# CovertLab/Lens

Measured on AMD Instinct MI355X. Metric: agent-steps/sec (whole node) at 1M agents; FP64 % peak; stencil HBM GB/s, higher is better.
Workload: dtype f64; 1 GPU; BASELINE config 4: 1M agents + 4096x4096 diffusion_field lattice; agents=1000000, agents_end=1000000, agents_start=1000000, integrator=dopri5, exchange=sorted, parallelism=row-bands x1, agents_in_bin_order=True, coupled_passes=False, stencil_mode=fma, halo=0

## Files before the change

include/vk_kinetics.h:

```cpp
#ifndef VK_KINETICS_H
#define VK_KINETICS_H

#include <stdint.h>

#ifdef __cplusplus
extern "C" {
#endif

#define VK_ABI_VERSION 1

typedef void *vk_stream_t;
typedef struct vk_table vk_table;

enum vk_status {
    VK_OK = 0,
    VK_ERR_ARG = 1,
    VK_ERR_HIP = 2,
    VK_ERR_LIMIT = 3,
    VK_ERR_NOMEM = 4
};

enum vk_agent_status {
    VK_AGENT_OK = 0,
    VK_AGENT_MAX_STEPS = 1,
// ... 69 lines not shown
int vk_step_dopri5_multi(const vk_table *t, int64_t n_agents, int64_t ld, double dt, int32_t n_steps,
                         const vk_ode_opts *opts, const double *params, double *conc, const double *m2c,
                         double *h_state, double *flux, int64_t step_flux, int64_t *counts,
                         int64_t step_counts, int32_t *status, int32_t *nsteps, int64_t step_nsteps,
                         vk_stream_t stream);


#define VK_UNIFORM_BLOCKS 512
int vk_field_uniform(const double *fields, int32_t n_fields, int64_t field_stride,
                     int32_t ny, int32_t row_lo, int32_t row_hi, double *summary,
                     int32_t *scratch, vk_stream_t stream);

int vk_diffuse(double *field, double *work0, double *work1, int32_t n_fields,
               int64_t field_stride, int32_t ny, int32_t row_lo, int32_t row_hi,
               int32_t lo_min, int32_t hi_max, int32_t edge_top, int32_t edge_bot,
               int32_t sub_begin, int32_t sub_count, int32_t n_sub, double coeff_dt,
               const double *uniform, vk_stream_t stream);

enum { VK_PART_ALL = 0, VK_PART_INTERIOR = 1, VK_PART_EDGES = 2 };
int vk_diffuse_part(double *field, double *work0, double *work1, int32_t n_fields,
                    int64_t field_stride, int32_t ny, int32_t row_lo, int32_t row_hi,
                    int32_t lo_min, int32_t hi_max, int32_t edge_top, int32_t edge_bot,
                    int32_t sub_begin, int32_t sub_count, int32_t n_sub, double coeff_dt,
                    const double *uniform, int32_t part, int32_t interior_passes,
                    vk_stream_t stream);

int vk_diffuse_delta(double *field, double *work0, double *work1, double *delta, int32_t n_fields,
                     int64_t field_stride, int32_t ny, int32_t row_lo, int32_t row_hi, int32_t lo_min,
                     int32_t hi_max, int32_t edge_top, int32_t edge_bot, int32_t sub_begin,
                     int32_t sub_count, int32_t n_sub, double coeff_dt, const double *uniform,
                     vk_stream_t stream);

int vk_diffuse_coupled(double *field, double *work0, double *work1, int32_t n_fields,
                       int64_t field_stride, int32_t ny, int32_t rows, int32_t n_sub, double coeff_dt,
                       const double *uniform, const int32_t *bin_lin, const int32_t *seg, int32_t nseg,
                       int64_t n_agents, const int32_t *gather_row, double *conc, int64_t conc_ld,
                       const int32_t *count_row, const int64_t *counts, int64_t counts_ld,
                       double binvol_avogadro, vk_stream_t stream);

enum { VK_BUF_FIELD = 0, VK_BUF_WORK0 = 1, VK_BUF_WORK1 = 2 };
enum { VK_PASS_SINGLE = 0, VK_PASS_WL3, VK_PASS_WL6, VK_PASS_WL6NT, VK_PASS_PS, VK_PASS_PS10,
       VK_PASS_PS10_ALIGNED, VK_PASS_PS10_STRIPS, VK_PASS_SP };
enum { VK_PLAN_COUPLED = 1, VK_PLAN_COUPLED_AGENTS = 2 };
typedef struct vk_pass {
    int32_t k, src, dst, f0;
    int32_t lo, hi, in_lo, in_hi, gap_lo, gap_hi;
    int32_t kernel, couple, copy_back;
} vk_pass;
int vk_diffuse_plan(int32_t row_lo, int32_t row_hi, int32_t lo_min, int32_t hi_max, int32_t edge_top,
                    int32_t edge_bot, int32_t sub_begin, int32_t sub_count, int32_t n_sub, int32_t part,
                    int32_t interior_passes, int32_t coupled, vk_pass *out, int32_t capacity,
                    int32_t *n_passes);

int vk_set_stencil_depth(int32_t k);

int vk_set_stencil_kernel(int32_t variant, int32_t rows);

int vk_set_stencil_mode(int32_t mode);

int vk_timestamp(uint64_t *out, int32_t idx, vk_stream_t stream);

int vk_copy_stream(const double *src, double *dst, int64_t n, vk_stream_t stream);

int64_t vk_wall_clock_khz(void);

int vk_gather(const double *fields, int64_t field_stride, const int32_t *bin_lin,
              int64_t n_agents, const int32_t *map_field, const int32_t *map_row,
              int32_t n_map, double *dst, int64_t ld, vk_stream_t stream);

int vk_exchange_sorted(double *fields, int64_t field_stride, const int32_t *occ_bin,
                       const int32_t *occ_ptr, const int32_t *occ_agent, int32_t n_occ,
                       const int64_t *counts, int64_t ld, const int32_t *map_count,
                       const int32_t *map_field, int32_t n_map, double binvol_avogadro,
                       vk_stream_t stream);

int vk_exchange_atomic(double *fields, int64_t field_stride, const int32_t *bin_lin,
                       int64_t n_agents, const int64_t *counts, int64_t ld,
                       const int32_t *map_count, const int32_t *map_field, int32_t n_map,
                       double binvol_avogadro, vk_stream_t stream);

int vk_bin_sites(const double *loc, int64_t n_agents, int64_t ld, int32_t nx, int32_t ny,
                 double bound_x, double bound_y, int32_t row_offset, int32_t *bin_lin,
                 int32_t *ix_out, vk_stream_t stream);


enum vk_cell_row {
    VK_CELL_MASS = 0,
    VK_CELL_VOLUME = 1,
    VK_CELL_LENGTH = 2,
    VK_CELL_SURFACE_AREA = 3,
    VK_CELL_PROTEIN = 4,
    VK_CELL_ANGLE = 5,
    VK_CELL_ROWS = 6
};

enum vk_growth_model {
    VK_GROWTH_PROTEIN = 0,
    VK_GROWTH_MASS = 1
};

enum vk_rng {
    VK_RNG_STREAM = 0,
    VK_RNG_PHILOX = 1
};

typedef struct vk_cell_params {
// ... 312 lines not shown
```

lens_amd/csrc/vk_lattice.hip:

```cpp

#include <math.h>
#include <stdint.h>

#include <algorithm>
#include <utility>
#include <vector>


#include "vk_bin.h"
#include "vk_internal.h"
#include "vk_pass_plan.h"
#include "vk_stencil_launch.h"

constexpr int ST_BX = 256;
constexpr int ST_RB = 16;

__global__ __launch_bounds__(ST_BX) void k_diffuse_substep(const double *__restrict__ src,
                                                           double *dst,
                                                           const double *f0,
                                                           int64_t field_stride, int ny, int lo, int hi,
                                                           int top_reflect, int bot_reflect, double coef,
                                                           const double *__restrict__ uniform, int delta_mode) {
    const int f = blockIdx.z;
    const int j = blockIdx.x * ST_BX + threadIdx.x;
    const int r0 = lo + blockIdx.y * ST_RB;
    if (j >= ny || r0 >= hi) return;
    const int r1 = min(r0 + ST_RB, hi);
    const double *s = src + (int64_t)f * field_stride;
    double *d = dst + (int64_t)f * field_stride;
    const double *g = f0 ? f0 + (int64_t)f * field_stride : nullptr;
    if (uniform && uniform[2 * f] == uniform[2 * f + 1]) {
        if (delta_mode)
            for (int r = r0; r < r1; ++r) d[(int64_t)r * ny + j] = 0.0;
        return;
    }
    const int jl = j > 0 ? j - 1 : 0;
    const int jr = j < ny - 1 ? j + 1 : ny - 1;
    const int ru = (r0 == top_reflect) ? r0 : r0 - 1;
    double up = s[(int64_t)ru * ny + j];
    double c = s[(int64_t)r0 * ny + j];
    for (int r = r0; r < r1; ++r) {
        const int rd = (r == bot_reflect) ? r : r + 1;
        const double down = s[(int64_t)rd * ny + j];
        const double left = s[(int64_t)r * ny + jl];
        const double right = s[(int64_t)r * ny + jr];
        const double lap = (((up + left) + (-4.0 * c)) + right) + down;
        double v = c + coef * lap;
        if (g) {
            const double base = g[(int64_t)r * ny + j];
            v = delta_mode ? v - base : base + (v - base);
        }
        d[(int64_t)r * ny + j] = v;
        up = c;
        c = down;
    }
}

// ... 25 lines not shown
    return prev;
}


__global__ void k_timestamp(uint64_t *out, int idx) {
    if (threadIdx.x == 0) out[idx] = wall_clock64();
}

extern "C" int vk_timestamp(uint64_t *out, int32_t idx, vk_stream_t stream) {
    if (!out || idx < 0) {
        vk::set_error("vk_timestamp: bad arguments");
        return VK_ERR_ARG;
    }
    hipLaunchKernelGGL(k_timestamp, dim3(1), dim3(64), 0, (hipStream_t)stream, out, idx);
    return vk::launch_check("k_timestamp");
}

typedef double vk_d2v __attribute__((ext_vector_type(2)));
__global__ __launch_bounds__(256) void k_copy_stream(const vk_d2v *__restrict__ s, vk_d2v *__restrict__ d, int64_t n) {
    const int64_t i = (int64_t)blockIdx.x * 256 + threadIdx.x;
    if (i < n) __builtin_nontemporal_store(s[i], d + i);
}

extern "C" int vk_copy_stream(const double *src, double *dst, int64_t n_doubles, vk_stream_t stream) {
    if (!src || !dst || n_doubles < 0 || (n_doubles & 1) || (((uintptr_t)src | (uintptr_t)dst) & 15)) {
        vk::set_error("vk_copy_stream: bad arguments (16-B aligned buffers of an even number of doubles)");
        return VK_ERR_ARG;
    }
    const int64_t n = n_doubles / 2;
    if (n == 0) return VK_OK;
    hipLaunchKernelGGL(k_copy_stream, dim3((unsigned)((n + 255) / 256)), dim3(256), 0, (hipStream_t)stream,
                       (const vk_d2v *)src, (vk_d2v *)dst, n);
    return vk::launch_check("k_copy_stream");
}

extern "C" int64_t vk_wall_clock_khz(void) {
    int dev = 0, khz = 0;
    if (hipGetDevice(&dev) != hipSuccess) return 0;
    if (hipDeviceGetAttribute(&khz, hipDeviceAttributeWallClockRate, dev) != hipSuccess) return 0;
    return khz;
}

__global__ __launch_bounds__(256) void k_copy_rows(const double *__restrict__ src, double *dst,
                                                   int64_t field_stride, int64_t off, int64_t count,
                                                   const double *__restrict__ uniform) {
    const int f = blockIdx.y;
    if (uniform && uniform[2 * f] == uniform[2 * f + 1]) return;
    const int64_t base = (int64_t)f * field_stride + off;
    for (int64_t i = (int64_t)blockIdx.x * blockDim.x + threadIdx.x; i < count; i += (int64_t)gridDim.x * blockDim.x)
        dst[base + i] = src[base + i];
}


static vk_plan::Settings stencil_settings() {
    return {g_stencil_mode, g_stencil_depth, g_stencil_kernel, g_stencil_rows};
}

struct PassArgs {
    double *buf[3];
    int nf;
    int64_t fs;
    int ny, top, bot, tile_rows;
    double coef;
    const double *uniform;
    const VkPsCouple *cp;
    hipStream_t stream;
};

static void launch_pass(const vk_pass &p, const PassArgs &a) {
    typedef void (*launcher)(VK_STENCIL_LAUNCH_ARGS);
    static const launcher launchers[] = {nullptr,        vk_launch_wl3,  vk_launch_wl6,          vk_launch_wl6nt,
                                         vk_launch_ps,   vk_launch_ps10, vk_launch_ps10_aligned, nullptr,
                                         vk_launch_sp};
    const double *src = a.buf[p.src], *f0 = p.f0 ? a.buf[VK_BUF_FIELD] : nullptr;
    double *dst = a.buf[p.dst];
    VkPsCouple c = {};
    if (a.cp) c = *a.cp, c.mode = p.couple;
    const VkPsCouple *cp = a.cp ? &c : nullptr;
    if (p.kernel == VK_PASS_SINGLE) {
        dim3 grid((a.ny + ST_BX - 1) / ST_BX, (p.hi - p.lo + ST_RB - 1) / ST_RB, a.nf);
        hipLaunchKernelGGL(k_diffuse_substep, grid, dim3(ST_BX), 0, a.stream, src, dst, f0, a.fs, a.ny, p.lo, p.hi, a.top,
                           a.bot, a.coef, a.uniform, 0);
    } else if (p.kernel == VK_PASS_PS10_STRIPS) {
        vk_launch_ps10_strips(p.k, a.stream, src, dst, f0, a.nf, a.fs, a.ny, p.lo, p.hi, p.in_lo, p.in_hi, a.top, a.bot,
                              a.coef, a.uniform, cp, a.tile_rows, p.gap_lo, p.gap_hi);
    } else {
        launchers[p.kernel](p.k, a.stream, src, dst, f0, a.nf, a.fs, a.ny, p.lo, p.hi, p.in_lo, p.in_hi, a.top, a.bot,
                            a.coef, a.uniform, cp, a.tile_rows);
    }
}

static int run_plan(const char *what, const vk_plan::Call &c, double *field, double *work0, double *work1, int32_t n_fields,
                    int64_t field_stride, int32_t ny, double coeff_dt, const double *uniform, const VkPsCouple *cp,
                    vk_stream_t stream) {
    const vk_plan::Settings st = stencil_settings();
    std::vector<vk_pass> passes;
    const char *why = "";
    int rc = vk_plan::plan(st, c, passes, &why);
    if (rc) {
        vk::set_error("%s: %s", what, why);
        return rc;
    }
    if (n_fields == 0) return VK_OK;
    const PassArgs a = {{field, work0, work1}, n_fields, field_stride, ny, c.edge_top ? c.lo_min : -1,
                        c.edge_bot ? c.hi_max - 1 : 0x7fffffff, st.rows, coeff_dt, uniform, cp, (hipStream_t)stream};
    for (const vk_pass &p : passes) {
        launch_pass(p, a);
        if ((rc = vk::launch_check(what))) return rc;
        if (p.copy_back) {
            const int64_t count = (int64_t)(c.row_hi - c.row_lo) * ny;
            const unsigned blocks = (unsigned)std::min<int64_t>(2048, (count + 255) / 256);
            hipLaunchKernelGGL(k_copy_rows, dim3(blocks, n_fields), dim3(256), 0, a.stream, work0, field, field_stride,
                               (int64_t)c.row_lo * ny, count, uniform);
            if ((rc = vk::launch_check("k_copy_rows"))) return rc;
        }
    }
    return VK_OK;
}

extern "C" int vk_diffuse_part(double *field, double *work0, double *work1, int32_t n_fields, int64_t field_stride,
                               int32_t ny, int32_t row_lo, int32_t row_hi, int32_t lo_min, int32_t hi_max,
                               int32_t edge_top, int32_t edge_bot, int32_t sub_begin, int32_t sub_count,
                               int32_t n_sub, double coeff_dt, const double *uniform, int32_t part,
                               int32_t interior_passes, vk_stream_t stream) {
    const vk_plan::Call c = {row_lo,    row_hi,    lo_min, hi_max, edge_top,        edge_bot,
                             sub_begin, sub_count, n_sub,  part,   interior_passes, 0};
    if (part != VK_PART_ALL && part != VK_PART_INTERIOR && part != VK_PART_EDGES) {
        vk::set_error("vk_diffuse_part: part must be VK_PART_ALL / _INTERIOR / _EDGES");
        return VK_ERR_ARG;
    }
    if (!field || n_fields < 0 || ny <= 0 || !vk_plan::geometry_ok(c) || (int64_t)hi_max * ny > field_stride) {
        vk::set_error("vk_diffuse: bad geometry");
        return VK_ERR_ARG;
    }
    if (!work0 || (n_sub > 2 && !work1)) {
        vk::set_error("vk_diffuse: work buffers required");
        return VK_ERR_ARG;
    }
    return run_plan("vk_diffuse", c, field, work0, work1, n_fields, field_stride, ny, coeff_dt, uniform, nullptr, stream);
}

extern "C" int vk_diffuse(double *field, double *work0, double *work1, int32_t n_fields,
                          int64_t field_stride, int32_t ny, int32_t row_lo, int32_t row_hi, int32_t lo_min,
                          int32_t hi_max, int32_t edge_top, int32_t edge_bot, int32_t sub_begin,
                          int32_t sub_count, int32_t n_sub, double coeff_dt, const double *uniform,
                          vk_stream_t stream) {
    return vk_diffuse_part(field, work0, work1, n_fields, field_stride, ny, row_lo, row_hi, lo_min, hi_max, edge_top,
                           edge_bot, sub_begin, sub_count, n_sub, coeff_dt, uniform, VK_PART_ALL, 0, stream);
}

extern "C" int vk_diffuse_plan(int32_t row_lo, int32_t row_hi, int32_t lo_min, int32_t hi_max, int32_t edge_top,
                               int32_t edge_bot, int32_t sub_begin, int32_t sub_count, int32_t n_sub, int32_t part,
                               int32_t interior_passes, int32_t coupled, vk_pass *out, int32_t capacity,
                               int32_t *n_passes) {
    const vk_plan::Call c = {row_lo,    row_hi,    lo_min, hi_max, edge_top,        edge_bot,
                             sub_begin, sub_count, n_sub,  part,   interior_passes, coupled};
    const bool whole_step = row_lo == 0 && lo_min == 0 && row_hi == hi_max && sub_begin == 0 && sub_count == n_sub &&
                            part == VK_PART_ALL;
    if (!n_passes || capacity < 0 || (capacity > 0 && !out) || part < VK_PART_ALL || part > VK_PART_EDGES ||
        coupled < 0 || coupled > VK_PLAN_COUPLED_AGENTS || (coupled && !whole_step) || !vk_plan::geometry_ok(c)) {
        vk::set_error("vk_diffuse_plan: bad arguments");
        return VK_ERR_ARG;
    }
    std::vector<vk_pass> passes;
    const char *why = "";
    const int rc = vk_plan::plan(stencil_settings(), c, passes, &why);
    if (rc) vk::set_error("vk_diffuse_plan: %s", why);
    *n_passes = (int32_t)passes.size();
    std::copy_n(passes.begin(), std::min<size_t>(passes.size(), (size_t)capacity), out);
    return rc;
}

extern "C" int vk_diffuse_coupled(double *field, double *work0, double *work1, int32_t n_fields,
                                  int64_t field_stride, int32_t ny, int32_t rows, int32_t n_sub, double coeff_dt,
                                  const double *uniform, const int32_t *bin_lin, const int32_t *seg, int32_t nseg,
                                  int64_t n_agents, const int32_t *gather_row, double *conc, int64_t conc_ld,
                                  const int32_t *count_row, const int64_t *counts, int64_t counts_ld,
                                  double binvol_avogadro, vk_stream_t stream) {
    if (!field || !work0 || !work1 || n_fields < 1 || ny <= 0 || rows <= 0 || n_sub < 0 ||
        (int64_t)rows * ny > field_stride || (int64_t)rows * ny >= INT32_MAX || n_agents < 0 ||
        n_agents >= INT32_MAX || nseg != (ny + 15) / 16 || (n_agents > 0 && (!bin_lin || !seg)) || !gather_row ||
        !count_row) {
        vk::set_error("vk_diffuse_coupled: bad arguments");
        return VK_ERR_ARG;
    }
    VkPsCouple cp = {};
    cp.bins = bin_lin;
    cp.seg = seg;
    cp.nseg = nseg;
    cp.n = (int32_t)n_agents;
    cp.gdst = conc;
    cp.gld = conc_ld;
    cp.counts = counts;
    cp.cld = counts_ld;
    cp.bva = binvol_avogadro;
    if (n_fields > VK_COUPLE_MAX_FIELDS) {
        vk::set_error("vk_diffuse_coupled: at most 8 planes");
        return VK_ERR_LIMIT;
    }
    for (int f = 0; f < n_fields; ++f) {
        if (gather_row[f] >= 127 || count_row[f] >= 127 || (gather_row[f] >= 0 && (!conc || conc_ld < n_agents)) ||
            (count_row[f] >= 0 && (!counts || counts_ld < n_agents))) {
            vk::set_error("vk_diffuse_coupled: bad gather / count rows");
            return VK_ERR_ARG;
        }
        cp.grow[f] = (int8_t)(gather_row[f] < 0 ? -1 : gather_row[f]);
        cp.crow[f] = (int8_t)(count_row[f] < 0 ? -1 : count_row[f]);
    }
    const vk_plan::Call c = {0, rows, 0, rows, 1, 1, 0, n_sub, n_sub, VK_PART_ALL, 0,
                             n_agents > 0 ? VK_PLAN_COUPLED_AGENTS : VK_PLAN_COUPLED};
    return run_plan("vk_diffuse_coupled", c, field, work0, work1, n_fields, field_stride, ny, coeff_dt, uniform, &cp, stream);
}

extern "C" int vk_diffuse_delta(double *field, double *work0, double *work1, double *delta, int32_t n_fields,
                                int64_t field_stride, int32_t ny, int32_t row_lo, int32_t row_hi, int32_t lo_min,
                                int32_t hi_max, int32_t edge_top, int32_t edge_bot, int32_t sub_begin,
                                int32_t sub_count, int32_t n_sub, double coeff_dt, const double *uniform,
                                vk_stream_t stream) {
    if (!delta || sub_count < 1 || sub_begin + sub_count != n_sub) {
        vk::set_error("vk_diffuse_delta: needs a delta buffer and the call must end at the last substep");
        return VK_ERR_ARG;
    }
    if (sub_count > 1) {
// ... 234 lines not shown
```

lens_amd/csrc/vk_pass_plan.h:

```cpp
#pragma once

#include <stdint.h>

#include <algorithm>
#include <vector>

#include "vk_kinetics.h"

namespace vk_plan {

struct Settings {
    int mode;
    int depth;
    int kernel;
    int rows;
};

struct Call {
    int row_lo, row_hi, lo_min, hi_max, edge_top, edge_bot, sub_begin, sub_count, n_sub, part, interior_passes, coupled;
};

inline bool geometry_ok(const Call &c) {
    return c.row_lo >= c.lo_min && c.row_hi <= c.hi_max && c.row_lo < c.row_hi && c.sub_begin >= 0 && c.sub_count >= 0 &&
           c.sub_begin + c.sub_count <= c.n_sub;
}

inline std::vector<int> odd_depths(int set_depth, int sub_count) {
    const int depth = set_depth == 10 ? 9 : std::min(set_depth | 1, 15);
    int passes = (sub_count + depth - 1) / depth;
    if ((passes & 1) != (sub_count & 1)) ++passes;
    std::vector<int> ks;
    for (int j = 0, left = passes; j < sub_count; --left) {
        const int rem = sub_count - j;
        int k = (rem + left - 1) / left;
        if ((k & 1) == 0) ++k;
        if (k > depth) k = depth;
        while (k > 1 && rem - k < left - 1) k -= 2;
        ks.push_back(k);
        j += k;
    }
    return ks;
}

inline int kernel_of(const Settings &s, int k, bool base, int couple, bool strip) {
    if (k == 1) return VK_PASS_SINGLE;
    if (s.mode == 1 && k <= 11 && ((k & 1) || k == 10)) {
        if (k != 10) return VK_PASS_PS;
        if (s.kernel == 40 && !strip && !couple) return VK_PASS_SP;
        return s.kernel == 70 && !strip ? VK_PASS_PS10_ALIGNED : VK_PASS_PS10;
    }
    if (k == 10 || ((s.kernel == 6 || s.kernel >= 20) && (k == 7 || k == 9 || k == 11))) return VK_PASS_WL6NT;
    return (s.kernel == 2 || base) ? VK_PASS_WL3 : VK_PASS_WL6;
}

inline int state_buffer(int j) { return j == 0 ? VK_BUF_FIELD : VK_BUF_WORK0 + ((j - 1) & 1); }

inline std::vector<int> ten_deep_buffers(const Settings &s, const Call &c, int P) {
    const bool ends_step = c.sub_begin + c.sub_count == c.n_sub;
    const int S = state_buffer(c.sub_begin);
    const int T = ends_step ? VK_BUF_FIELD : state_buffer(c.sub_begin + c.sub_count);
    const int cand[3] = {VK_BUF_WORK0, VK_BUF_WORK1, VK_BUF_FIELD};
    const int nc = (ends_step && s.mode == 1) ? 3 : 2;
    std::vector<int> dsts(P, -1);
    dsts[P - 1] = T;
    for (int p = P - 2; p >= 0; --p) {
        for (int i = 0; i < nc && dsts[p] < 0; ++i)
            if (cand[i] != dsts[p + 1] && (p > 0 || cand[i] != S)) dsts[p] = cand[i];
        if (dsts[p] < 0) return {};
// ... 21 lines not shown
        p.gap_lo = gap_lo, p.gap_hi = gap_hi;
        if (c.coupled == VK_PLAN_COUPLED_AGENTS)
            p.couple = (e - k + 1 == 0 ? 1 : 0) | (e == c.n_sub - 1 ? 2 : 0);
        p.kernel = gap_lo >= 0 ? VK_PASS_PS10_STRIPS : kernel_of(s, k, base, p.couple, strip);
        out.push_back(p);
    };
    const int P = c.sub_count / 10;
    std::vector<int> dsts;
    if (ten_block && P <= 64 && (!c.coupled || (s.mode == 1 && P >= 2))) dsts = ten_deep_buffers(s, c, P);
    if (!dsts.empty()) {
        const int m = (c.interior_passes <= 0 || c.interior_passes > P) ? P : c.interior_passes;
        for (int p = 0; p < P; ++p) {
            if (c.part == VK_PART_INTERIOR && p >= m) break;
            const int e = c.sub_begin + 10 * p + 9, grow = last - e;
            const int lo = std::max(c.lo_min, c.row_lo - grow), hi = std::min(c.hi_max, c.row_hi + grow);
            const int src = p ? dsts[p - 1] : state_buffer(c.sub_begin);
            const bool base = (s.mode != 1 || c.coupled) && ends_step && p == P - 1;
            const int ilo = halo_top ? c.row_lo + 10 * (p + 1) : lo, ihi = halo_bot ? c.row_hi - 10 * (p + 1) : hi;
            if (c.part == VK_PART_ALL || (c.part == VK_PART_EDGES && p >= m)) {
                add(10, e, src, dsts[p], base, lo, hi, false, -1, -1);
            } else if (c.part == VK_PART_INTERIOR) {
                if (ilo < ihi) add(10, e, src, dsts[p], base, ilo, ihi, false, -1, -1);
            } else if (halo_top && halo_bot && ilo < ihi && s.mode == 1) {
                add(10, e, src, dsts[p], base, lo, hi, true, ilo, ihi);
            } else {
                if (halo_top && lo < ilo) add(10, e, src, dsts[p], base, lo, ilo, true, -1, -1);
                if (halo_bot && ihi < hi) add(10, e, src, dsts[p], base, ihi, hi, true, -1, -1);
            }
        }
        return VK_OK;
    }
    if (c.part != VK_PART_ALL) {
        *why = "no 10-deep buffer plan for this block";
        return VK_ERR_LIMIT;
    }
    const std::vector<int> ks = odd_depths(s.depth, c.sub_count);
    if (c.coupled && (ks.size() < 2 || *std::min_element(ks.begin(), ks.end()) < 2)) {
        *why = "the step is not planned as two or more fused passes";
        return VK_ERR_LIMIT;
    }
    int j = c.sub_begin;
    for (int k : ks) {
        const int e = j + k - 1, grow = last - e;
        const bool final_pass = e == c.n_sub - 1, in_place = final_pass && j == 0;
        const int dst = in_place ? VK_BUF_WORK0 : (final_pass ? VK_BUF_FIELD : state_buffer(e + 1));
        add(k, e, state_buffer(j), dst, final_pass, std::max(c.lo_min, c.row_lo - grow),
            std::min(c.hi_max, c.row_hi + grow), false, -1, -1);
        out.back().copy_back = in_place;
        j += k;
    }
    return VK_OK;
}

}
```

lens_amd/lattice.py:

```python

from __future__ import annotations

import ctypes
from typing import Callable, Optional, Sequence

import torch

from lens_amd import native

N_A_LEGACY = 6.022140857e23


def n_substeps(timestep: float, dt_max: float = 0.01) -> int:
    t, dt, n = 0.0, min(timestep, dt_max), 0
    while t < timestep:
        t += dt
        n += 1
    return n


def whole_plane(lat) -> bool:
    return not (lat.pad_top or lat.pad_bot or not (lat.edge_top and lat.edge_bot))


def stencil_depth(k: int = 0) -> int:
    native.load()
    return native._lib.vk_set_stencil_depth(int(k))


def stencil_kernel(variant: int = -1, rows: int = -1) -> int:
    native.load()
    if int(variant) != -1 and int(variant) not in STENCIL_VARIANTS:
        raise ValueError('stencil kernel %d is not built (variants: %s)' % (variant, sorted(STENCIL_VARIANTS)))
    if int(rows) != -1 and not (int(rows) == 0 or 8 <= int(rows) <= 4096):
        raise ValueError('stencil tile rows must be 0 (auto) or 8..4096, got %d' % rows)
    return native._lib.vk_set_stencil_kernel(int(variant), int(rows))


STENCIL_VARIANTS = frozenset((2, 3, 6, 20, 40, 70))


def stencil_mode(mode=None) -> str:
    native.load()
    names = ('exact', 'fma')
    code = -1 if mode is None else names.index(mode)
    return names[native._lib.vk_set_stencil_mode(code)]


class Lattice:
    def __init__(self, molecules: Sequence[str], n_bins, bounds, depth: float, diffusion: float,
                 device=None, row_band=None, halo: int = 0, avogadro: float = N_A_LEGACY,
                 initial=None):
        native.load()
        self.molecules = list(molecules)
        self.n_bins = [int(n_bins[0]), int(n_bins[1])]
        self.bounds = [float(bounds[0]), float(bounds[1])]
        self.depth = float(depth)
        self.avogadro = float(avogadro)
        nx, ny = self.n_bins
        self.device = native.resolve_device(device)
        dx = self.bounds[0] / nx
        dy = self.bounds[1] / ny
        self.diffusion = diffusion / (dx * dy)
        self.diffusion_dt = 0.01
        self.bin_volume = (self.depth * self.bounds[0] * self.bounds[1]) * 1e-15 / (nx * ny)
        self.binvol_avogadro = self.bin_volume * self.avogadro
        lo, hi = (0, nx) if row_band is None else (int(row_band[0]), int(row_band[1]))
        if not (0 <= lo < hi <= nx):
            raise ValueError('bad row band %r' % (row_band,))
        self.row_lo_global, self.row_hi_global = lo, hi
        self.halo = int(halo)
        self.edge_top = lo == 0
        self.edge_bot = hi == nx
        if not (self.edge_top and self.edge_bot) and self.halo < 1:
            raise ValueError('a row band %r of %d rows needs halo >= 1 (got %d)' % ((lo, hi), nx, self.halo))
        if self.halo > hi - lo and not (self.edge_top and self.edge_bot):
            raise ValueError('halo (%d) deeper than the band (%d rows)' % (self.halo, hi - lo))
        h = self.halo
        self.pad_top = 0 if self.edge_top else h
        self.pad_bot = 0 if self.edge_bot else h
        self.rows_local = self.pad_top + (hi - lo) + self.pad_bot
        self.ny = ny
        nf = len(self.molecules)
        shape = (nf, self.rows_local, ny)
        self.fields = torch.zeros(shape, dtype=torch.float64, device=self.device)
        self.work0 = torch.empty(shape, dtype=torch.float64, device=self.device)
        self.work1 = torch.empty(shape, dtype=torch.float64, device=self.device)
        self.uniform = torch.empty(2 * max(nf, 1), dtype=torch.float64, device=self.device)
        self._uniform_scratch = torch.empty(max(nf, 1) * native.VK_UNIFORM_BLOCKS, dtype=torch.int32,
                                            device=self.device)
        if initial is not None:
            for f, m in enumerate(self.molecules):
                if m in initial:
                    self.set_field(m, initial[m])
        else:
            self.fields.fill_(1.0)

    @property
    def row_lo(self) -> int:
# ... 256 lines not shown
```

lens_amd/native.py:

```python

from __future__ import annotations

import ctypes
import os

import numpy as np

LIB_DIR = os.path.join(os.path.dirname(os.path.abspath(__file__)), 'lib')
LIB_PATH = os.environ.get('VK_KINETICS_LIB') or os.path.join(LIB_DIR, 'libvk_kinetics.so')

VK_OK, VK_ERR_ARG, VK_ERR_HIP, VK_ERR_LIMIT, VK_ERR_NOMEM = 0, 1, 2, 3, 4
VK_AGENT_MAX_STEPS, VK_AGENT_H_UNDERFLOW, VK_AGENT_NONFINITE = 1, 2, 4

EXPORTS = (
    'vk_abi_version', 'vk_last_error', 'vk_table_create', 'vk_table_destroy', 'vk_table_specialize',
    'vk_rate_fluxes', 'vk_step_euler', 'vk_step_dopri5', 'vk_step_dopri5_multi', 'vk_step_dopri5_gather', 'vk_field_uniform',
    'vk_diffuse', 'vk_diffuse_part', 'vk_diffuse_delta', 'vk_diffuse_coupled', 'vk_diffuse_plan', 'vk_set_stencil_depth', 'vk_set_stencil_kernel', 'vk_set_stencil_mode',
    'vk_timestamp', 'vk_wall_clock_khz', 'vk_copy_stream', 'vk_gather', 'vk_exchange_sorted',
    'vk_exchange_atomic', 'vk_bin_sites', 'vk_cell_step', 'vk_divide_scratch_bytes', 'vk_divide_plan',
    'vk_divide_gather', 'vk_divide_lineage', 'vk_divide_locations', 'vk_kremling_step',
    'vk_expression_step', 'vk_motility_step', 'vk_occupancy_scratch_bytes', 'vk_occupancy_sort',
    'vk_exchange_ordered', 'vk_contact_scratch_bytes', 'vk_contact_step',
    'vk_response_begin', 'vk_response_end', 'vk_response_cells', 'vk_exchange_ordered_mixed',
    'vk_exchange_atomic_f64', 'vk_population_scratch_bytes', 'vk_population_plan', 'vk_contact_step_channels',
    'vk_flagella_step', 'vk_flagella_counts', 'vk_divide_flagella',
    'vk_ssa_step', 'vk_ssa_propensities', 'vk_divide_counts', 'vk_ssa_flagella_target',
)

VK_CELL_MASS, VK_CELL_VOLUME, VK_CELL_LENGTH, VK_CELL_SURFACE_AREA, VK_CELL_PROTEIN, VK_CELL_ANGLE = range(6)
VK_CELL_ROWS = 6
(VK_MOTIL_N_METHYL, VK_MOTIL_ACTIVITY, VK_MOTIL_CHEY_P, VK_MOTIL_CCW_MOTOR_BIAS, VK_MOTIL_CCW_TO_CW,
 VK_MOTIL_MOTOR_STATE, VK_MOTIL_ANGLE, VK_MOTIL_THRUST, VK_MOTIL_TORQUE) = range(9)
VK_MOTIL_ROWS = 9
VK_FLAG_CHEY, VK_FLAG_CHEY_P, VK_FLAG_CW_BIAS, VK_FLAG_MOTILE_STATE, VK_FLAG_PMF = range(5)
VK_FLAG_ROWS = 5
VK_FLAGI_TARGET, VK_FLAGI_HAVE, VK_FLAGI_MASK = range(3)
VK_FLAGI_ROWS = 3
VK_FLAGELLA_MERGED, VK_FLAGELLA_SPLIT_DICT = 0, 1
VK_DIVIDE_FLAGELLA_DOMAIN = 0x666c6167656c6c61
VK_SSA_MAX_SPECIES, VK_SSA_MAX_REACTIONS, VK_SSA_MAX_ORDER = 64, 32, 255
VK_SSA_DOMAIN = 0x7373615f73746570
VK_SSA_DIVIDE_DOMAIN = 0x7373615f64697669
VK_SSA_MAX_EVENTS, VK_SSA_NONFINITE, VK_SSA_OVERFLOW, VK_SSA_BAD_KEY = 1, 2, 4, 8
VK_GROWTH_PROTEIN, VK_GROWTH_MASS = 0, 1
VK_RNG_STREAM, VK_RNG_PHILOX = 0, 1
VK_DIVIDE_SET, VK_DIVIDE_SPLIT, VK_DIVIDE_ZERO = 0, 1, 2
VK_UNIFORM_BLOCKS = 512
VK_PART_ALL, VK_PART_INTERIOR, VK_PART_EDGES = 0, 1, 2
VK_PLAN_COUPLED, VK_PLAN_COUPLED_AGENTS = 1, 2


class NativeError(RuntimeError):
    pass


_i32p = ctypes.POINTER(ctypes.c_int32)
_f64p = ctypes.POINTER(ctypes.c_double)
_vp = ctypes.c_void_p
_i32 = ctypes.c_int32
_i64 = ctypes.c_int64
_f64 = ctypes.c_double


class VkTableDesc(ctypes.Structure):
    _fields_ = [(n, ctypes.c_int32) for n in (
        'n_species', 'n_dyn', 'n_reactions', 'n_rate_laws', 'n_params', 'n_ext',
        'n_sets', 'n_members', 'n_upd', 'n_exch')] + [
        ('rl_reaction', _i32p), ('rl_enzyme', _i32p), ('rl_kcat', _i32p),
        ('rl_num_ptr', _i32p), ('rl_den_ptr', _i32p), ('set_ptr', _i32p),
        ('mem_species', _i32p), ('mem_param', _i32p), ('upd_ptr', _i32p),
# ... 37 lines not shown
class VkContactParams(ctypes.Structure):
    _fields_ = [(n, ctypes.c_int32) for n in ('iterations', 'gx', 'gy', 'reserved')] + [
        (n, ctypes.c_double) for n in ('stiffness', 'max_length', 'width', 'length', 'max_push', 'max_turn',
                                       'jitter', 'jitter_angle')] + [('seed', ctypes.c_uint64)]


class VkContactChannels(ctypes.Structure):
    _fields_ = [(n, ctypes.c_double) for n in ('height', 'space', 'spacer')] + [
        ('n_lines', ctypes.c_int32), ('reserved', ctypes.c_int32)]


class VkResponseTable(ctypes.Structure):
    _fields_ = [(n, ctypes.c_int32) for n in ('n_mol', 'n_porin', 'n_det', 'n_save', 'n_expr', 'n_flux', 'n_ext',
                                              'reserved')] + [
        (n, _vp) for n in ('mol_int_row', 'mol_ext_row', 'porin_row', 'porin_perm', 'det_row', 'det_thr',
                           'save_row', 'expr_row')] + [('avogadro', ctypes.c_double), ('volume_fl', ctypes.c_double)]


class VkSsaNet(ctypes.Structure):
    _fields_ = [(n, ctypes.c_int32) for n in ('n_species', 'n_reactions', 'max_order', 'n_inv')] + [
        (n, _vp) for n in ('react_ptr', 'react_species', 'react_order', 'stoich_ptr', 'stoich_species',
                           'stoich_delta', 'rates', 'inv')]


class VkPass(ctypes.Structure):
    _fields_ = [(n, ctypes.c_int32) for n in ('k', 'src', 'dst', 'f0', 'lo', 'hi', 'in_lo', 'in_hi', 'gap_lo',
                                              'gap_hi', 'kernel', 'couple', 'copy_back')]


_SIGS = {
    'vk_abi_version': ([], ctypes.c_int),
    'vk_last_error': ([], ctypes.c_char_p),
    'vk_table_create': ([ctypes.POINTER(VkTableDesc), ctypes.POINTER(_vp)], ctypes.c_int),
    'vk_table_destroy': ([_vp], ctypes.c_int),
    'vk_table_specialize': ([_vp, ctypes.c_char_p], ctypes.c_int),
    'vk_rate_fluxes': ([_vp, _i64, _i64, _vp, _vp, _vp, _vp], ctypes.c_int),
    'vk_step_euler': ([_vp, _i64, _i64, _f64, _vp, _vp, _vp, _vp, _vp, _vp, _vp, _vp], ctypes.c_int),
    'vk_step_dopri5': ([_vp, _i64, _i64, _f64, ctypes.POINTER(VkOdeOpts), _vp, _vp, _vp, _vp,
                        _vp, _vp, _vp, _vp, _vp, _vp], ctypes.c_int),
    'vk_step_dopri5_multi': ([_vp, _i64, _i64, _f64, _i32, ctypes.POINTER(VkOdeOpts), _vp, _vp, _vp, _vp, _vp,
                              _i64, _vp, _i64, _vp, _vp, _i64, _vp], ctypes.c_int),
    'vk_step_dopri5_gather': ([_vp, _i64, _i64, _f64, ctypes.POINTER(VkOdeOpts), _vp, _vp, _vp, _vp, _vp, _vp,
                               _vp, _vp, _vp, _i64, _vp, _vp, _vp, _i32, _vp], ctypes.c_int),
    'vk_field_uniform': ([_vp, _i32, _i64, _i32, _i32, _i32, _vp, _vp, _vp], ctypes.c_int),
    'vk_diffuse': ([_vp, _vp, _vp, _i32, _i64, _i32, _i32, _i32, _i32, _i32, _i32, _i32,
                    _i32, _i32, _i32, _f64, _vp, _vp], ctypes.c_int),
    'vk_diffuse_part': ([_vp, _vp, _vp, _i32, _i64, _i32, _i32, _i32, _i32, _i32, _i32, _i32,
                         _i32, _i32, _i32, _f64, _vp, _i32, _i32, _vp], ctypes.c_int),
    'vk_diffuse_delta': ([_vp, _vp, _vp, _vp, _i32, _i64, _i32, _i32, _i32, _i32, _i32, _i32, _i32,
                          _i32, _i32, _i32, _f64, _vp, _vp], ctypes.c_int),
    'vk_diffuse_coupled': ([_vp, _vp, _vp, _i32, _i64, _i32, _i32, _i32, _f64, _vp, _vp, _vp, _i32, _i64,
                            _i32p, _vp, _i64, _i32p, _vp, _i64, _f64, _vp], ctypes.c_int),
    'vk_diffuse_plan': ([_i32] * 12 + [ctypes.POINTER(VkPass), _i32, _i32p], ctypes.c_int),
    'vk_set_stencil_depth': ([_i32], ctypes.c_int),
    'vk_set_stencil_kernel': ([_i32, _i32], ctypes.c_int),
    'vk_set_stencil_mode': ([_i32], ctypes.c_int),
    'vk_timestamp': ([_vp, _i32, _vp], ctypes.c_int),
    'vk_wall_clock_khz': ([], ctypes.c_int64),
    'vk_copy_stream': ([_vp, _vp, _i64, _vp], ctypes.c_int),
    'vk_gather': ([_vp, _i64, _vp, _i64, _vp, _vp, _i32, _vp, _i64, _vp], ctypes.c_int),
    'vk_exchange_sorted': ([_vp, _i64, _vp, _vp, _vp, _i32, _vp, _i64, _vp, _vp, _i32, _f64, _vp],
                           ctypes.c_int),
    'vk_exchange_atomic': ([_vp, _i64, _vp, _i64, _vp, _i64, _vp, _vp, _i32, _f64, _vp], ctypes.c_int),
    'vk_bin_sites': ([_vp, _i64, _i64, _i32, _i32, _f64, _f64, _i32, _vp, _vp, _vp], ctypes.c_int),
    'vk_cell_step': ([ctypes.POINTER(VkCellParams), _i64, _i64, _vp, _vp, _vp, _vp, _vp, _vp, _vp, _vp],
                     ctypes.c_int),
    'vk_divide_scratch_bytes': ([_i64], ctypes.c_int64),
    'vk_divide_plan': ([_vp, _i64, _vp, _vp, _vp, _vp, _vp], ctypes.c_int),
    'vk_divide_gather': ([_i64, _vp, _vp, _vp, _i64, _vp, _i64, _i32, _i32, _i32, _vp], ctypes.c_int),
    'vk_divide_lineage': ([_i64, _vp, _vp, _vp, _vp, _vp, _vp, _vp, _vp, _vp, _vp], ctypes.c_int),
    'vk_divide_locations': ([_i64, _vp, _vp, _vp, _i64, _vp, _i64, _vp, _vp], ctypes.c_int),
    'vk_expression_step': ([_vp, _i64, _i64, _f64, _vp, _vp, _vp, _i32, _vp], ctypes.c_int),
    'vk_kremling_step': ([ctypes.POINTER(VkKremlingParams), _i64, _i64, _f64, _f64, _i32, _f64, _f64, _i32,
                          _vp, _vp, _f64, _vp, _vp, _vp, _vp, _vp, _vp], ctypes.c_int),
    'vk_motility_step': ([ctypes.POINTER(VkMotilityParams), _i64, _i64, _f64, _i32, _vp, _vp, _vp, _vp, _i32, _i32,
                          _f64, _f64, _vp, _vp, _vp, _vp], ctypes.c_int),
    'vk_flagella_step': ([ctypes.POINTER(VkMotilityParams), ctypes.POINTER(VkFlagellaParams), _i64, _i64, _f64, _i32,
                          _vp, _vp, _vp, _vp, _vp, _vp, _i32, _i32, _f64, _f64, _vp, _vp, _vp, _vp], ctypes.c_int),
    'vk_flagella_counts': ([_i64, _vp, _vp, _vp, _vp, _vp], ctypes.c_int),
    'vk_divide_flagella': ([_i64, _i64, _i64, _vp, _vp, _vp, _i64, _vp, _vp, _vp, _vp, _vp, _i64, _vp, _i32,
                            ctypes.c_uint64, ctypes.c_uint64, _i64, _vp], ctypes.c_int),
    'vk_ssa_step': ([ctypes.POINTER(VkSsaNet), _i64, _i64, _f64, _vp, _vp, ctypes.c_uint64, _vp, _i32, _vp, _vp, _vp],
                    ctypes.c_int),
    'vk_ssa_propensities': ([ctypes.POINTER(VkSsaNet), _i64, _i64, _vp, _vp, _vp], ctypes.c_int),
    'vk_divide_counts': ([_i64, _i64, _i64, _vp, _vp, _vp, _i64, _vp, _vp, _i64, _vp, _i32, ctypes.c_uint64,
                          ctypes.c_uint64, _i64, _vp], ctypes.c_int),
    'vk_ssa_flagella_target': ([_i64, _vp, _vp, _vp, _vp], ctypes.c_int),
    'vk_occupancy_scratch_bytes': ([_i64], ctypes.c_int64),
    'vk_occupancy_sort': ([_vp, _vp, _i64, _i64, _vp, _vp, _vp, _i64, _vp], ctypes.c_int),
    'vk_exchange_ordered': ([_vp, _i64, _vp, _vp, _i64, _vp, _i64, _vp, _vp, _i32, _f64, _vp], ctypes.c_int),
    'vk_contact_scratch_bytes': ([_i64, _i64], ctypes.c_int64),
    'vk_contact_step': ([ctypes.POINTER(VkContactParams), _i64, _i64, _vp, _vp, _vp, _vp, _vp, _vp, _i32, _i32,
                         _f64, _f64, _vp, _vp, _vp, _i64, _vp], ctypes.c_int),
    'vk_contact_step_channels': ([ctypes.POINTER(VkContactParams), _i64, _i64, _vp, _vp, _vp, _vp, _vp, _vp, _i32,
                                  _i32, _f64, _f64, _vp, _vp, _vp, _i64, ctypes.POINTER(VkContactChannels), _vp, _vp],
                                 ctypes.c_int),
    'vk_population_scratch_bytes': ([_i64], ctypes.c_int64),
    'vk_population_plan': ([_vp, _vp, _i64, _vp, _vp, _vp, _vp, _vp], ctypes.c_int),
    'vk_response_begin': ([ctypes.POINTER(VkResponseTable), _i64, _i64, _f64] + [_vp] * 14, ctypes.c_int),
    'vk_response_end': ([ctypes.POINTER(VkResponseTable), _i64, _i64] + [_vp] * 15, ctypes.c_int),
    'vk_response_cells': ([_i32, _i64, _i64, _vp, _vp, _vp, _vp, _vp, _vp, _vp, _vp, _vp], ctypes.c_int),
    'vk_exchange_ordered_mixed': ([_vp, _i64, _vp, _vp, _i64, _vp, _i64, _vp, _vp, _i32, _vp, _i64, _vp, _vp, _i32,
                                   _f64, _vp], ctypes.c_int),
    'vk_exchange_atomic_f64': ([_vp, _i64, _vp, _i64, _vp, _i64, _vp, _vp, _i32, _f64, _vp], ctypes.c_int),
}

# ... 94 lines not shown
```

Baseline: 793.7 million agent-steps/s.

## Split stencil passes into two row bands on a second stream with event dependencies

Adds a banded planning mode that splits each 10-step PS10 stencil pass into a top and a bottom row band. The bottom bands run on an extra non-blocking stream and wait on events from the previous top band, so the two bands' passes can overlap as a skewed wavefront. This targets the serialization and tail idle time between full-lattice passes on the whole-step 4096-row case. In exchange it adds event and stream overhead, extra halo-row reads at the band boundary, and a fallback path when graph capture or event limits prevent it.

```diff
diff --git a/include/vk_kinetics.h b/include/vk_kinetics.h
--- a/include/vk_kinetics.h
+++ b/include/vk_kinetics.h
@@ -145,6 +145,13 @@
                     int32_t interior_passes, int32_t coupled, vk_pass *out, int32_t capacity,
                     int32_t *n_passes);
 
+int vk_diffuse_plan_lanes(int32_t row_lo, int32_t row_hi, int32_t lo_min, int32_t hi_max, int32_t edge_top,
+                          int32_t edge_bot, int32_t sub_begin, int32_t sub_count, int32_t n_sub,
+                          int32_t part, int32_t interior_passes, int32_t coupled, vk_pass *out,
+                          int32_t *lane, int32_t *after, int32_t capacity, int32_t *n_passes);
+
+int vk_set_stencil_bands(int32_t bands, int32_t top_rows);
+
 int vk_set_stencil_depth(int32_t k);
 
 int vk_set_stencil_kernel(int32_t variant, int32_t rows);
diff --git a/lens_amd/csrc/vk_lattice.hip b/lens_amd/csrc/vk_lattice.hip
--- a/lens_amd/csrc/vk_lattice.hip
+++ b/lens_amd/csrc/vk_lattice.hip
@@ -3,6 +3,7 @@
 #include <stdint.h>
 
 #include <algorithm>
+#include <mutex>
 #include <utility>
 #include <vector>
 
@@ -134,8 +135,51 @@
 }
 
 
+static int g_stencil_bands = 0;
+static int g_stencil_top_rows = 0;
+
+extern "C" int vk_set_stencil_bands(int32_t bands, int32_t top_rows) {
+    const int prev = g_stencil_bands;
+    if (bands == 0 || bands == 1 || (bands == 2 && top_rows > 0)) {
+        g_stencil_bands = bands;
+        g_stencil_top_rows = bands == 2 ? top_rows : 0;
+    }
+    return prev;
+}
+
 static vk_plan::Settings stencil_settings() {
-    return {g_stencil_mode, g_stencil_depth, g_stencil_kernel, g_stencil_rows};
+    return {g_stencil_mode, g_stencil_depth, g_stencil_kernel, g_stencil_rows, g_stencil_bands, g_stencil_top_rows};
+}
+
+constexpr int BAND_EVENTS = 66;
+struct BandLanes {
+    hipStream_t stream = nullptr;
+    hipEvent_t ev[BAND_EVENTS] = {};
+};
+static std::mutex g_band_mutex;
+static std::vector<BandLanes *> g_band_lanes;
+
+static BandLanes *band_lanes(hipStream_t caller) {
+    int dev = 0;
+    if (hipGetDevice(&dev) != hipSuccess || dev < 0) return nullptr;
+    std::lock_guard<std::mutex> lock(g_band_mutex);
+    if ((size_t)dev >= g_band_lanes.size()) g_band_lanes.resize(dev + 1, nullptr);
+    if (g_band_lanes[dev]) return g_band_lanes[dev];
+    hipStreamCaptureStatus cap = hipStreamCaptureStatusNone;
+    if (hipStreamIsCapturing(caller, &cap) != hipSuccess || cap != hipStreamCaptureStatusNone) return nullptr;
+    BandLanes *l = new BandLanes;
+    bool ok = hipStreamCreateWithFlags(&l->stream, hipStreamNonBlocking) == hipSuccess;
+    for (int i = 0; ok && i < BAND_EVENTS; ++i) ok = hipEventCreateWithFlags(&l->ev[i], hipEventDisableTiming) == hipSuccess;
+    if (!ok) {
+        for (hipEvent_t e : l->ev)
+            if (e) (void)hipEventDestroy(e);
+        if (l->stream) (void)hipStreamDestroy(l->stream);
+        delete l;
+        (void)hipGetLastError();
+        return nullptr;
+    }
+    g_band_lanes[dev] = l;
+    return l;
 }
 
 struct PassArgs {
@@ -175,17 +219,47 @@
 static int run_plan(const char *what, const vk_plan::Call &c, double *field, double *work0, double *work1, int32_t n_fields,
                     int64_t field_stride, int32_t ny, double coeff_dt, const double *uniform, const VkPsCouple *cp,
                     vk_stream_t stream) {
-    const vk_plan::Settings st = stencil_settings();
+    vk_plan::Settings st = stencil_settings();
     std::vector<vk_pass> passes;
+    std::vector<int32_t> lane, after;
     const char *why = "";
-    int rc = vk_plan::plan(st, c, passes, &why);
+    int rc = vk_plan::plan_lanes(st, c, passes, lane, after, &why);
     if (rc) {
         vk::set_error("%s: %s", what, why);
         return rc;
     }
     if (n_fields == 0) return VK_OK;
-    const PassArgs a = {{field, work0, work1}, n_fields, field_stride, ny, c.edge_top ? c.lo_min : -1,
-                        c.edge_bot ? c.hi_max - 1 : 0x7fffffff, st.rows, coeff_dt, uniform, cp, (hipStream_t)stream};
+    const bool banded = std::find(lane.begin(), lane.end(), 1) != lane.end();
+    BandLanes *bl = banded ? band_lanes((hipStream_t)stream) : nullptr;
+    std::vector<int> slot(passes.size(), -1);
+    int slots = 0;
+    for (int32_t i : after)
+        if (i >= 0 && slot[i] < 0) slot[i] = slots++;
+    if (banded && (!bl || slots + 2 > BAND_EVENTS)) {
+        st.bands = 1;
+        bl = nullptr;
+        if ((rc = vk_plan::plan_lanes(st, c, passes, lane, after, &why))) return rc;
+    }
+    PassArgs a = {{field, work0, work1}, n_fields, field_stride, ny, c.edge_top ? c.lo_min : -1,
+                  c.edge_bot ? c.hi_max - 1 : 0x7fffffff, st.rows, coeff_dt, uniform, cp, (hipStream_t)stream};
+    if (bl) {
+        hipStream_t lanes[2] = {(hipStream_t)stream, bl->stream};
+        hipEvent_t fork = bl->ev[BAND_EVENTS - 2], join = bl->ev[BAND_EVENTS - 1];
+        if ((rc = vk::hip_check(hipEventRecord(fork, lanes[0]), what))) return rc;
+        if ((rc = vk::hip_check(hipStreamWaitEvent(lanes[1], fork, 0), what))) return rc;
+        int failed = VK_OK;
+        for (size_t i = 0; i < passes.size() && !failed; ++i) {
+            a.stream = lanes[lane[i]];
+            if (after[i] >= 0) failed = vk::hip_check(hipStreamWaitEvent(a.stream, bl->ev[slot[after[i]]], 0), what);
+            if (failed) break;
+            launch_pass(passes[i], a);
+            failed = vk::launch_check(what);
+            if (!failed && slot[i] >= 0) failed = vk::hip_check(hipEventRecord(bl->ev[slot[i]], a.stream), what);
+        }
+        rc = vk::hip_check(hipEventRecord(join, lanes[1]), what);
+        if (!rc) rc = vk::hip_check(hipStreamWaitEvent(lanes[0], join, 0), what);
+        return failed ? failed : rc;
+    }
     for (const vk_pass &p : passes) {
         launch_pass(p, a);
         if ((rc = vk::launch_check(what))) return rc;
@@ -231,10 +305,10 @@
                            edge_bot, sub_begin, sub_count, n_sub, coeff_dt, uniform, VK_PART_ALL, 0, stream);
 }
 
-extern "C" int vk_diffuse_plan(int32_t row_lo, int32_t row_hi, int32_t lo_min, int32_t hi_max, int32_t edge_top,
-                               int32_t edge_bot, int32_t sub_begin, int32_t sub_count, int32_t n_sub, int32_t part,
-                               int32_t interior_passes, int32_t coupled, vk_pass *out, int32_t capacity,
-                               int32_t *n_passes) {
+extern "C" int vk_diffuse_plan_lanes(int32_t row_lo, int32_t row_hi, int32_t lo_min, int32_t hi_max, int32_t edge_top,
+                                     int32_t edge_bot, int32_t sub_begin, int32_t sub_count, int32_t n_sub,
+                                     int32_t part, int32_t interior_passes, int32_t coupled, vk_pass *out,
+                                     int32_t *lane, int32_t *after, int32_t capacity, int32_t *n_passes) {
     const vk_plan::Call c = {row_lo,    row_hi,    lo_min, hi_max, edge_top,        edge_bot,
                              sub_begin, sub_count, n_sub,  part,   interior_passes, coupled};
     const bool whole_step = row_lo == 0 && lo_min == 0 && row_hi == hi_max && sub_begin == 0 && sub_count == n_sub &&
@@ -245,12 +319,24 @@
         return VK_ERR_ARG;
     }
     std::vector<vk_pass> passes;
+    std::vector<int32_t> lanes, afters;
     const char *why = "";
-    const int rc = vk_plan::plan(stencil_settings(), c, passes, &why);
+    const int rc = vk_plan::plan_lanes(stencil_settings(), c, passes, lanes, afters, &why);
     if (rc) vk::set_error("vk_diffuse_plan: %s", why);
     *n_passes = (int32_t)passes.size();
-    std::copy_n(passes.begin(), std::min<size_t>(passes.size(), (size_t)capacity), out);
+    const size_t n = std::min<size_t>(passes.size(), (size_t)capacity);
+    std::copy_n(passes.begin(), n, out);
+    if (lane) std::copy_n(lanes.begin(), n, lane);
+    if (after) std::copy_n(afters.begin(), n, after);
     return rc;
+}
+
+extern "C" int vk_diffuse_plan(int32_t row_lo, int32_t row_hi, int32_t lo_min, int32_t hi_max, int32_t edge_top,
+                               int32_t edge_bot, int32_t sub_begin, int32_t sub_count, int32_t n_sub, int32_t part,
+                               int32_t interior_passes, int32_t coupled, vk_pass *out, int32_t capacity,
+                               int32_t *n_passes) {
+    return vk_diffuse_plan_lanes(row_lo, row_hi, lo_min, hi_max, edge_top, edge_bot, sub_begin, sub_count, n_sub, part,
+                                 interior_passes, coupled, out, nullptr, nullptr, capacity, n_passes);
 }
 
 extern "C" int vk_diffuse_coupled(double *field, double *work0, double *work1, int32_t n_fields,
diff --git a/lens_amd/csrc/vk_pass_plan.h b/lens_amd/csrc/vk_pass_plan.h
--- a/lens_amd/csrc/vk_pass_plan.h
+++ b/lens_amd/csrc/vk_pass_plan.h
@@ -14,6 +14,8 @@
     int depth;
     int kernel;
     int rows;
+    int bands;
+    int top_rows;
 };
 
 struct Call {
@@ -141,4 +143,39 @@
     return VK_OK;
 }
 
+inline int auto_top_rows(const Call &c, const std::vector<vk_pass> &passes) {
+    if (c.row_hi - c.row_lo != 4096 || passes.size() != 10) return 0;
+    for (const vk_pass &p : passes)
+        if (p.kernel != VK_PASS_PS10_ALIGNED) return 0;
+    return 2 * 4096 / 5;
 }
+
+inline int plan_lanes(const Settings &s, const Call &c, std::vector<vk_pass> &out, std::vector<int32_t> &lane,
+                      std::vector<int32_t> &after, const char **why) {
+    const int rc = plan(s, c, out, why);
+    lane.assign(out.size(), 0);
+    after.assign(out.size(), -1);
+    if (rc != VK_OK || s.bands == 1 || out.empty()) return rc;
+    const bool whole_step = c.part == VK_PART_ALL && c.edge_top && c.edge_bot && c.row_lo == c.lo_min &&
+                            c.row_hi == c.hi_max && c.sub_begin == 0 && c.sub_count == c.n_sub && !c.coupled;
+    if (!whole_step) return rc;
+    for (const vk_pass &p : out)
+        if (p.k != 10 || (p.kernel != VK_PASS_PS10 && p.kernel != VK_PASS_PS10_ALIGNED) || p.copy_back) return rc;
+    const int P = (int)out.size(), N = c.row_hi - c.row_lo;
+    const int m0 = s.bands == 2 ? s.top_rows : auto_top_rows(c, out);
+    if (m0 - 10 * (P - 1) < 10 || m0 >= N) return rc;
+    std::vector<vk_pass> banded;
+    lane.clear(), after.clear();
+    for (int p = 0; p < P; ++p) {
+        const int m = c.row_lo + m0 - 10 * p;
+        vk_pass t = out[p], b = out[p];
+        t.hi = m, t.in_hi = std::min(c.hi_max, m + 10);
+        b.lo = m, b.in_lo = std::max(c.lo_min, m - 10);
+        banded.push_back(t), lane.push_back(0), after.push_back(-1);
+        banded.push_back(b), lane.push_back(1), after.push_back(p ? 2 * (p - 1) : -1);
+    }
+    out.swap(banded);
+    return rc;
+}
+
+}
diff --git a/lens_amd/lattice.py b/lens_amd/lattice.py
--- a/lens_amd/lattice.py
+++ b/lens_amd/lattice.py
@@ -45,6 +45,15 @@
     names = ('exact', 'fma')
     code = -1 if mode is None else names.index(mode)
     return names[native._lib.vk_set_stencil_mode(code)]
+
+
+def stencil_bands(bands: int = -1, top_rows: int = 0) -> int:
+    native.load()
+    if int(bands) not in (-1, 0, 1, 2):
+        raise ValueError('stencil bands must be 0 (auto), 1 (off) or 2 (forced), got %d' % bands)
+    if int(bands) == 2 and int(top_rows) <= 0:
+        raise ValueError('forced stencil bands need the top band\'s rows, got %d' % top_rows)
+    return native._lib.vk_set_stencil_bands(int(bands), int(top_rows))
 
 
 class Lattice:
diff --git a/lens_amd/native.py b/lens_amd/native.py
--- a/lens_amd/native.py
+++ b/lens_amd/native.py
@@ -15,7 +15,7 @@
 EXPORTS = (
     'vk_abi_version', 'vk_last_error', 'vk_table_create', 'vk_table_destroy', 'vk_table_specialize',
     'vk_rate_fluxes', 'vk_step_euler', 'vk_step_dopri5', 'vk_step_dopri5_multi', 'vk_step_dopri5_gather', 'vk_field_uniform',
-    'vk_diffuse', 'vk_diffuse_part', 'vk_diffuse_delta', 'vk_diffuse_coupled', 'vk_diffuse_plan', 'vk_set_stencil_depth', 'vk_set_stencil_kernel', 'vk_set_stencil_mode',
+    'vk_diffuse', 'vk_diffuse_part', 'vk_diffuse_delta', 'vk_diffuse_coupled', 'vk_diffuse_plan', 'vk_diffuse_plan_lanes', 'vk_set_stencil_bands', 'vk_set_stencil_depth', 'vk_set_stencil_kernel', 'vk_set_stencil_mode',
     'vk_timestamp', 'vk_wall_clock_khz', 'vk_copy_stream', 'vk_gather', 'vk_exchange_sorted',
     'vk_exchange_atomic', 'vk_bin_sites', 'vk_cell_step', 'vk_divide_scratch_bytes', 'vk_divide_plan',
     'vk_divide_gather', 'vk_divide_lineage', 'vk_divide_locations', 'vk_kremling_step',
@@ -159,6 +159,8 @@
     'vk_diffuse_coupled': ([_vp, _vp, _vp, _i32, _i64, _i32, _i32, _i32, _f64, _vp, _vp, _vp, _i32, _i64,
                             _i32p, _vp, _i64, _i32p, _vp, _i64, _f64, _vp], ctypes.c_int),
     'vk_diffuse_plan': ([_i32] * 12 + [ctypes.POINTER(VkPass), _i32, _i32p], ctypes.c_int),
+    'vk_diffuse_plan_lanes': ([_i32] * 12 + [ctypes.POINTER(VkPass), _i32p, _i32p, _i32, _i32p], ctypes.c_int),
+    'vk_set_stencil_bands': ([_i32, _i32], ctypes.c_int),
     'vk_set_stencil_depth': ([_i32], ctypes.c_int),
     'vk_set_stencil_kernel': ([_i32, _i32], ctypes.c_int),
     'vk_set_stencil_mode': ([_i32], ctypes.c_int),
```

Measured after the change: 847.8 million agent-steps/s (median of 6 runs). +6.8%, better.
